# shamim-hussain/egt

Hardware: AMD Instinct MI355X
Metric: graphs/sec EGT fwd+bwd, ZINC-500K padded N=64 (higher is better)
Workload: dtype f32; 1 GPU; zinc500k_n64: attention-block stack (h,e,mask)->(h',e') x Ly, fwd+bwd + param grads; scope=stack, graphs_per_gpu=128, global_batch=128, N=64, Dh=64, De=64, H=8, d=8, Ly=10, parallelism=dp1, grad_allreduce_bytes=740480, backend=none (single process), flat_grad_adopted=True, flat_grad_bound=True, collective_in_graph=False

## Files before the change

egt_amd/csrc/egt_block.hip:

```cpp
#include "egt_common.h"

#include <stdlib.h>
#include <string.h>
#include <vector>

#include "egt_block.h"
#include "egt_tile.h"

#include "egt_block_dev.h"
#include "egt_dma.h"

#include "egt_block_fwd.h"
#include "egt_block_bwd.h"



struct EgtBlockEnv {
  bool no_narrow_fwd, no_narrow_bwd;
  int bwd_mm;
  int bwd_tl, fwd_rows;
  int nrw_fwd_waves, nrw_bwd_waves, nrw_fwd_half;
};
static bool env_flag_raw(const char* name) {
  const char* v = getenv(name);
// ... 109 lines not shown
    P.fwd_nw = r4 ? 4 : 8;
    P.fl = {B * ((N + 4 * P.fwd_nw - 1) / (4 * P.fwd_nw)), 64 * P.fwd_nw, r4 ? lds_r4 : lds_r8};
  } else {
    P.fwd = FwdKernel::tile;
    P.fl = {B * ((N + P.RGF - 1) / P.RGF), 256, lds_tiles + (P.kvl ? lds_kv : 0)};
  }
  P.epi_ok = P.fwd != FwdKernel::tile || P.kvl;

  if (E.bwd_tl >= 4 && E.bwd_tl <= BWD_TL) P.TL = E.bwd_tl;
  else if (DE != 8) {
    const int g = tg > groups ? tg : groups;
    P.TL = (N + g - 1) / g;
  } else if (B * groups <= cus) {
    P.TL = BWD_TL;
    if (N > 8)
      for (int tl = 8; tl < BWD_TL; ++tl)
        if (B * ((N + tl - 1) / tl) <= cus) { P.TL = tl; break; }
  } else P.TL = (N + groups - 1) / groups;
  P.NLR = (N + P.TL - 1) / P.TL;
  P.nwg_bwd = B * P.NLR;
  P.EP = GG::EP;
  if (DE == 8 && !ml && !E.no_narrow_bwd) {
    P.bwd = BwdKernel::narrow;
    P.bwd_nw = E.nrw_bwd_waves == 8 || (E.nrw_bwd_waves != 4 && P.nwg_bwd <= cus && N >= 64) ? 8 : 4;
    P.bl = {P.nwg_bwd, 64 * P.bwd_nw, egt_narrow_bwd_lds(P.bwd_nw)};
  } else if (DE <= 16 && !ml) {
    constexpr int PWR = V4R_RR * (2 * GG::TILE_FLOATS + 256 + 192);
    P.bwd = BwdKernel::v4r;
    P.bl = {P.nwg_bwd, 256,
            ((size_t)(4 * PWR > BWD_PRO_WS ? 4 * PWR : BWD_PRO_WS) + (size_t)BWD_TL * QD_LD + 3 * GG::TILES * 256 + 3 * 2048 + 4) * 4};
  } else if (DE >= 32 && !ml && d->dtype != EGT_BF16) {
    P.bwd = BwdKernel::v5;
    P.mm = E.bwd_mm;
    P.bl = {P.nwg_bwd, 256, ((size_t)V5_AREA(DE) + (size_t)BWD_TL * QD_LD + 3 * ((GG::TILES + 1) / 2) * 512 + 4) * 4};
  } else {
    constexpr int PW = 3 * GG::TILE_FLOATS + 256 + 192;
    P.bwd = BwdKernel::v4;
    P.bl = {P.nwg_bwd, 256,
            ((size_t)(4 * PW > BWD_PRO_WS ? 4 * PW : BWD_PRO_WS) + (size_t)BWD_TL * QD_LD + 3 * ((GG::TILES + 1) / 2) * 512) * 4};
  }

  const size_t rows = (size_t)B * N;
  const int Dh = d->d * d->H;
  size_t o = 0;
  P.v_att = o; o += al(rows * Dh);
  P.stats = o; o += al(rows * BH * 4);
  P.qkvp = o; o += al(rows * QKVP);
  P.pw_sv = o; o += al((size_t)GG::DEP * 16 + 16);
  P.wfrag_sv = o; o += al(Dh <= 64 ? WFRAG_FLOATS : 0);
  P.saved_total = o;
  o = 0;
  P.dvp = o; o += al(rows * 64);
  P.dqp_sz = al(rows * 64 * (size_t)groups);
  P.dkvp_sz = al((size_t)P.nwg_bwd * N * 128);
  P.dqp = o; o += 2 * P.dqp_sz;
  P.dkvp = o; o += 2 * P.dkvp_sz;
  P.common_total = o;
  o = 0;
  P.pw = o; o += al((size_t)GG::DEP * 16 + 16);
  P.epart = o; o += al((size_t)P.nwg_bwd * P.EP);
  {
    const int node_wg = B * ((N + NODE_RC - 1) / NODE_RC);
    const size_t nmax = (size_t)(P.nwg_bwd > node_wg ? P.nwg_bwd : node_wg);
    P.spart = o; o += al(nmax * (5 * Dh));
    P.sbo = o; o += al(nmax * Dh);
  }
  P.wpart = o; o += al((size_t)egt_node_wgrad_chunks((int)rows, 1) * (Dh * 3 * Dh + Dh * Dh));
// ... 158 lines not shown
static int launch_fwd(BlockArgs& a, const BlockPlan& P, hipStream_t st, bool skip_pre) {
  if (!skip_pre) egt_node_launch_pre(a, st);
  if (!(P.epi_ok && node_fused_ok(a))) a.epi = 0;
  a.guard = 0;
  a.RGF = P.RGF;
  switch (P.fwd) {
    case FwdKernel::narrow: egt_narrow_launch_fwd(a, P.fwd_nw, P.fwd_half, P.fl, st); break;
    case FwdKernel::r4:
      if constexpr (DE <= 16) { if (a.bf16) launch_r4<DE, true>(a, P, st); else launch_r4<DE, false>(a, P, st); }
      break;
    case FwdKernel::tile: if (a.bf16) launch_tile_fwd<DE, true>(a, P, st); else launch_tile_fwd<DE, false>(a, P, st); break;
  }
  if (a.epi == 0) egt_node_launch_post(a, st);
  return a.epi;
}

template <int DE>
static void launch_bwd(BlockArgs& a, const BlockPlan& P, hipStream_t st, bool top, BlockArgs* below, BlockArgs* above, bool fuse) {
  static_assert(DE % 16 == 0 || DE == 8, "edge widths of the pair kernels");
  const bool pro = fuse;
  a.pro = 0;
  if (pro) {
    a.pro = top ? 1 : 2;
    a.sbo_n = P.nwg_bwd;
    if (!top) {
      a.up_h = above->h; a.up_nm_g = above->nm_g; a.up_Wqkv = above->Wqkv; a.up_wfrag = above->wfrag; a.up_dh_out = above->dh_out;
      a.up_dqp = above->dqp; a.up_dkvp = above->dkvp; a.up_dqkv_sv = above->dqkv_sv; a.up_spart = above->spart;
      above->spart_n = P.nwg_bwd;
    }
    if (a.prep) egt_node_launch_prep(&a, 1, st);
  } else if (top) {
    egt_node_launch_bwd(a, &a, false, st);
  }
  a.NQP = (a.N + 15) / 16;
  a.guard = 0;
  switch (P.bwd) {
    case BwdKernel::narrow: egt_narrow_launch_bwd(a, P.bwd_nw, P.bl, st); break;
    case BwdKernel::v4r:
      if constexpr (DE <= 16) {
        if (a.bf16) egt_launch_planned<k_block_bwd_v4r<DE, true, V4R_RR>>("k_block_bwd", P.bl, st, a);
        else egt_launch_planned<k_block_bwd_v4r<DE, false, V4R_RR>>("k_block_bwd", P.bl, st, a);
      }
      break;
    case BwdKernel::v5:
      if constexpr (DE >= 32) launch_v5<DE>(a, P, st);
      break;
    case BwdKernel::v4: if (a.bf16) launch_v4<DE, true>(a, P, st); else launch_v4<DE, false>(a, P, st); break;
  }
  if (!pro) egt_node_launch_bwd(a, below, true, st);
  else if (!below) egt_node_launch_bwd(a, nullptr, true, st);
}


extern "C" int egt_block_fwd(const egt_block_desc* desc, const egt_block_params* params,
                             const void* h, const void* e, const uint8_t* key_mask,
                             const void* attn_mask, const uint8_t* rand_mask, void* h_out,
                             void* e_out, void* saved, void* workspace, void* stream) {
  BlockArgs a;
  int rc = fill_block(desc, params, a);
  if (rc) return rc;
  if (!h || !e || !h_out || !e_out || !saved || !workspace)
    EGT_FAIL(EGT_E_NULL, "h/e/h_out/e_out/saved/workspace is NULL");
  if ((desc->flags & EGT_BF_ATTN_MASK) && !attn_mask) EGT_FAIL(EGT_E_NULL, "ATTN_MASK set but attn_mask is NULL");
  const BlockPlan P = plan_block(desc, mask_tensor(desc, rand_mask));
  bind_common(desc, P, a, h, e, key_mask, attn_mask, rand_mask, (float*)saved, (float*)workspace);
  a.h_out = (float*)h_out; a.e_out = (float*)e_out;
  a.epi = 1;
// ... 165 lines not shown
```

egt_amd/csrc/egt_block_bwd.h:

```cpp
#pragma once
#ifndef EGT_NT_BWD_E
#define EGT_NT_BWD_E true
#endif
#ifndef EGT_NT_BWD_DY
#define EGT_NT_BWD_DY false
#endif
#ifndef EGT_NT_BWD_ST
#define EGT_NT_BWD_ST false
#endif

template <int DE, bool ML, bool BF, bool RAG>
__global__ void __launch_bounds__(256, 2) k_block_bwd_v4(BlockArgs a) {
  seed_from_device(a);
  using G = Geo<DE>;
  typedef typename EdgeT<BF>::type ET;
  const ET* e_in = reinterpret_cast<const ET*>(a.e);
  ET* e_o = reinterpret_cast<ET*>(a.e_out);
  const ET* dey_in = reinterpret_cast<const ET*>(a.de_out);
  ET* dex_o = reinterpret_cast<ET*>(a.de);
  (void)e_in; (void)e_o; (void)dey_in; (void)dex_o;
  extern __shared__ __attribute__((aligned(16))) float sm[];
  const int lane = threadIdx.x & 63, wave = threadIdx.x >> 6;
  const int p = lane & 15, q = lane >> 4;
  const int N = a.N, TL = a.TL;
// ... 281 lines not shown
  constexpr int NS = (Geo<DE>::TILES + 1) / 2;
  (void)SPLIT; (void)NS;
  using G = Geo<DE>;
  const float* e_in = a.e;
  const float* dey_in = a.de_out;
  float* dex_o = a.de;
  extern __shared__ __attribute__((aligned(16))) float sm[];
  const int lane = threadIdx.x & 63, wave = __builtin_amdgcn_readfirstlane(threadIdx.x >> 6);
  const int p = lane & 15, q = lane >> 4;
  const int N = a.N, TL = a.TL;
  const int wg = a.xcd ? egt_xcd_remap(blockIdx.x, gridDim.x) : (int)blockIdx.x;
  const int b = wg / a.NLR, lr = wg % a.NLR;
  const int l_begin = lr * TL, l_end = min(N, l_begin + TL), nl = l_end - l_begin;
  const bool gated = (a.flags & EGT_BF_GATE) != 0;
  const bool clip = (a.flags & EGT_BF_CLIP) != 0;
  constexpr int PW = 3 * G::TILE_FLOATS + 256 + 192;
  constexpr int WSLAB = (MM != 0 && NS * 512 > G::TILES * 256) ? NS * 512 : G::TILES * 256;
  constexpr int PW2 = 2 * G::TILE_FLOATS + 256 + 192;
  float* et0 = sm + wave * G::TILE_FLOATS;
  float* et1 = sm + 4 * G::TILE_FLOATS + wave * PW2;
  const int estr = __builtin_amdgcn_readfirstlane((int)(et1 - et0));
  float* dt = et1 + G::TILE_FLOATS;
  float* sc1 = dt + G::TILE_FLOATS;
  float* sc2 = sc1 + 256;
  constexpr int AREA = V5_AREA(DE);
  static_assert(4 * PW == 4 * G::TILE_FLOATS + 4 * PW2 && AREA >= 4 * PW && AREA >= 4 * G::TILE_FLOATS + BWD_PRO_WS, "tile area");
  float* pro_ws = sm + 4 * G::TILE_FLOATS;
  float* qd = sm + AREA;
  float* wsA = qd + TL * QD_LD;
  float* wsB = wsA + WSLAB;
  float* wsD = wsB + WSLAB;
  volatile int* pflag = reinterpret_cast<volatile int*>(wsD + WSLAB);
  if (threadIdx.x < 4) pflag[threadIdx.x] = 0;
  const unsigned et_lds = __builtin_amdgcn_readfirstlane((unsigned)(size_t)et0);
  const unsigned off0 = dma_lane_offset<DE>(lane);
  const int ntile = RAG ? (N + 15) / 16 : N / 16;
  const bool balance = RAG && V5_BALANCE && ntile >= 3 && (ntile & 3) != 0;
  const int T_ = ntile * nl;
  const int t0 = balance ? (wave * T_) >> 2 : 0, t1 = balance ? ((wave + 1) * T_) >> 2 : 0;
  const bool have = balance ? t1 > t0 : wave < ntile;
  const int mt_first = balance ? t0 / nl : wave, mt_last = balance ? (t1 - 1) / nl : ntile - 1, mt_step = balance ? 1 : 4;
  const int r0_first = balance ? t0 - mt_first * nl : 0;
  float Kf[16], Vf[16];
  int kmv = 1;
#define V5_TILE_START(MT_, ROW_)                                                                                    \
  do {                                                                                                              \
    const int m0_ = (MT_) * 16, kv_ = RAG ? min(16, N - m0_) : 16;                                                  \
    if (RAG && kv_ < 16) tile_dma_ragged<DE>(et_lds, e_in + (((size_t)b * N + l_begin + (ROW_)) * N + m0_) * DE, lane, kv_); \
    else tile_dma<DE, EGT_NT_BWD_E>(et_lds, e_in + (((size_t)b * N + l_begin + (ROW_)) * N + m0_) * DE, off0);      \
    const size_t rowm_ = (size_t)b * N + (RAG ? min(m0_ + p, N - 1) : m0_ + p);                                     \
    const float4* kp_ = reinterpret_cast<const float4*>(a.qkvp + rowm_ * QKVP + 64 + q * 16);                       \
    const float4* vp_ = reinterpret_cast<const float4*>(a.qkvp + rowm_ * QKVP + 128 + q * 16);                      \
    _Pragma("unroll") for (int i = 0; i < 4; ++i) {                                                                 \
      const float4 kv4 = kp_[i], vv4 = vp_[i];                                                                      \
      Kf[4*i] = kv4.x; Kf[4*i+1] = kv4.y; Kf[4*i+2] = kv4.z; Kf[4*i+3] = kv4.w;                                     \
      Vf[4*i] = vv4.x; Vf[4*i+1] = vv4.y; Vf[4*i+2] = vv4.z; Vf[4*i+3] = vv4.w;                                     \
    }                                                                                                               \
    kmv = a.km ? (int)a.km[rowm_] : 1;                                                                              \
  } while (0)
  if (have) V5_TILE_START(mt_first, r0_first);
  BwdProRegs proR;
  {
    float4 sv[3];
#pragma unroll
    for (int u = 0; u < 3; ++u) {
      const int i = threadIdx.x + 256 * u, r = i / 40, f = i % 40;
// ... 40 lines not shown
    bwd_node_prologue_finish<DE>(a, pro_ws, qd, b, l_begin, wg, proR);
  }
  PSTAMP(1);
  if constexpr (MM != 0) {
    uint16_t* A16 = reinterpret_cast<uint16_t*>(wsA);
    uint16_t* B16 = reinterpret_cast<uint16_t*>(wsB);
    uint16_t* D16 = reinterpret_cast<uint16_t*>(wsD);
    auto parts = [](float v, uint16_t& hi, uint16_t& lo) {
      const uint32_t h = pk_bf16(v, 0.f) & 0xFFFFu;
      hi = (uint16_t)h;
      lo = (uint16_t)(pk_bf16(v - __uint_as_float(h << 16), 0.f) & 0xFFFFu);
    };
    for (int idx = threadIdx.x; idx < NS * 512; idx += 256) {
      const int i = idx & 7, ln = (idx >> 3) & 63, s_ = idx >> 9, pp = ln & 15, qq = ln >> 4, t = 2 * s_ + (i >> 2);
      const int c = 16 * t + 4 * qq + (i & 3);
      const bool in = t < G::TILES && c < DE;
      const int hd = 2 * (pp >> 2) + (pp & 1);
      uint16_t hi, lo;
      parts(in ? a.pw[c * 16 + pp] : 0.f, hi, lo);
      A16[((s_ * 2 + 0) * 64 + ln) * 8 + i] = hi; A16[((s_ * 2 + 1) * 64 + ln) * 8 + i] = lo;
      parts((in && (pp & 2) == 0) ? a.Wr[hd * DE + c] : 0.f, hi, lo);
      B16[((s_ * 2 + 0) * 64 + ln) * 8 + i] = hi; B16[((s_ * 2 + 1) * 64 + ln) * 8 + i] = lo;
    }
    for (int idx = threadIdx.x; idx < G::TILES * 256; idx += 256) {
      const int u = idx & 3, ln = (idx >> 2) & 63, t = idx >> 8, pp = ln & 15, qq = ln >> 4;
      uint16_t hi, lo;
      parts(a.pw[(16 * t + pp) * 16 + 4 * qq + u], hi, lo);
      D16[(t * 64 + ln) * 8 + u] = hi; D16[(t * 64 + ln) * 8 + 4 + u] = lo;
    }
  }
  float c2r[4];
#pragma unroll
  for (int r = 0; r < 4; ++r) c2r[r] = a.pw[G::DEP * 16 + 4 * q + r];

  v4f accT[G::TILES], accR[G::TILES];
#pragma unroll
  for (int t = 0; t < G::TILES; ++t) { accT[t] = (v4f){0.f, 0.f, 0.f, 0.f}; accR[t] = (v4f){0.f, 0.f, 0.f, 0.f}; }
  float ssum[4] = {0.f, 0.f, 0.f, 0.f};
  __syncthreads();
  PSTAMP(2);

  for (int mt = mt_first; have && mt <= mt_last; mt += mt_step) {
    const int r0 = (balance && mt == mt_first) ? r0_first : 0;
    const int r1 = (balance && mt == mt_last) ? t1 - mt * nl : nl;
    const int m0 = mt * 16, m = m0 + p;
    const int kv = RAG ? min(16, N - m0) : 16;
    const bool kvalid = RAG ? (p < kv) : true;
    if (mt != mt_first) V5_TILE_START(mt, r0);
    float dKa[16], dVa[16];
#pragma unroll
    for (int i = 0; i < 16; ++i) { dKa[i] = 0.f; dVa[i] = 0.f; }
    asm volatile("" : "+v"(kmv));
    const float kadd = kmv == 0 ? -EGT_NEG : 0.0f;
    const int l_first = l_begin + r0, l_stop = l_begin + r1;
    for (int l = l_first; l < l_stop; ++l) {
      const int li = l - l_begin;
      const int lj = l - l_first;
      const size_t rowl = (size_t)b * N + l;
      const size_t pair0 = rowl * N + m0;
      float* et = et0 + (lj & 1) * estr;
      MaskRegs mr{make_float2(1.f, 1.f), 0};
      TileRegs<DE> td;
      tile_gload<DE, EGT_NT_BWD_DY>(td, dey_in + pair0 * DE, lane, kv);
      if (lj == 0) vm_wait<(G::NF4 + 63) / 64>(); else vm_wait<2 * ((G::NF4 + 63) / 64) + 1>();
      SCHED_FENCE();
      float rstd;
      v4f acc = {c2r[0], c2r[1], c2r[2], c2r[3]};
      {
        float4 x[G::TILES];
#pragma unroll
        for (int t = 0; t < G::TILES; ++t) x[t] = frag_read<DE>(et, p, q, t);
        rstd = ln_frags<DE>(x, q, a.ln_eps, (a.flags & EGT_BF_NO_EDGE_LN) == 0);
        if constexpr (MM != 0) {
#pragma unroll
          for (int t = 0; t < G::TILES; ++t) frag_write<DE>(et, p, q, t, x[t]);
          v4f xv[G::TILES];
          Bf8 xh[NS], xl[NS];
#pragma unroll
          for (int t = 0; t < G::TILES; ++t) xv[t] = (v4f){x[t].x, x[t].y, x[t].z, x[t].w};
          split_tiles<G::TILES, SPLIT>(xv, xh, xl);
          acc = bf_gemm<NS, SPLIT>(wsA, 0, lane, xh, xl, acc);
        } else {
#pragma unroll
        for (int t = 0; t < G::TILES; ++t) {
          frag_write<DE>(et, p, q, t, x[t]);
          const float4 w = *reinterpret_cast<const float4*>(wsA + (t * 64 + lane) * 4);
          acc = MFMA(w.x, x[t].x, acc);
          acc = MFMA(w.y, x[t].y, acc);
          acc = MFMA(w.z, x[t].z, acc);
          acc = MFMA(w.w, x[t].w, acc);
        }
        }
      }
      SCHED_FENCE();
      tile_lds_put<DE>(dt, td, lane, kv);
      lds_sync();
      if (l + 1 < l_stop) {
        if (RAG && kv < 16) tile_dma_ragged<DE>(et_lds + (unsigned)(((lj + 1) & 1) * estr * 4), e_in + (pair0 + (size_t)N) * DE, lane, kv);
        else tile_dma<DE, EGT_NT_BWD_E>(et_lds + (unsigned)(((lj + 1) & 1) * estr * 4), e_in + (pair0 + (size_t)N) * DE, off0);
      }
// ... 44 lines not shown
        float xl[2], gl[2], inr[2];
#pragma unroll
        for (int j = 0; j < 2; ++j) {
          const float araw = dots[j] * a.scale;
          float ah = araw;
          inr[j] = 1.0f;
          if (clip) {
            inr[j] = (araw >= a.clip_lo && araw <= a.clip_hi) ? 1.0f : 0.0f;
            ah = fminf(fmaxf(araw, a.clip_lo), a.clip_hi);
          }
          hh[j] = ah + acc[2 * j + 1];
          xl[j] = hh[j];
          gl[j] = acc[2 * j];
        }
        apply_masks<false>(a, kadd, mr, (pair0 + p) * BH, q, xl, gl);
        if (RAG && !kvalid) { xl[0] = xl[1] = -3.0e38f; gl[0] = gl[1] = -3.0e38f; }
#pragma unroll
        for (int j = 0; j < 2; ++j) {
          const float S = __expf(xl[j] - st[4 * j]) * st[4 * j + 1];
          const float g = (gated || (RAG && !kvalid)) ? egt_sigmoid(gl[j]) : 1.0f;
          const float dS = dAd[j] * g;
          const float dGl = gated ? dAd[j] * S * g * (1.0f - g) : 0.f;
          const float dH = S * (dS - st[4 * j + 2]) + dhx[j];
          dA[j] = dH * inr[j] * a.scale;
          at[j] = S * g;
          dge[2 * j] = dGl;
          dge[2 * j + 1] = dH;
        }
      }
#pragma unroll
      for (int r = 0; r < 4; ++r) ssum[r] += dge[r];
      *reinterpret_cast<float4*>(sc1 + p * 16 + 4 * q) = make_float4(dge[0], dge[1], dge[2], dge[3]);
      *reinterpret_cast<float2*>(sc2 + p * 12 + 2 * q) = make_float2(hh[0], hh[1]);
      if (q == 0) sc2[p * 12 + 8] = 1.0f;
      lds_sync();
      SCHED_FENCE();
      if (!(a.guard & 4))
      {
        const float* qr = qd + li * QD_LD;
        const float4* qp = reinterpret_cast<const float4*>(qr + q * 16);
        const float4* dp = reinterpret_cast<const float4*>(qr + 64 + q * 16);
        float dq[16];
#pragma unroll
        for (int i = 0; i < 4; ++i) {
          const float4 u = qp[i], v = dp[i];
          dKa[4*i]   = fmaf(dA[0], u.x, dKa[4*i]);   dKa[4*i+1] = fmaf(dA[1], u.y, dKa[4*i+1]);
          dKa[4*i+2] = fmaf(dA[0], u.z, dKa[4*i+2]); dKa[4*i+3] = fmaf(dA[1], u.w, dKa[4*i+3]);
          dVa[4*i]   = fmaf(at[0], v.x, dVa[4*i]);   dVa[4*i+1] = fmaf(at[1], v.y, dVa[4*i+1]);
          dVa[4*i+2] = fmaf(at[0], v.z, dVa[4*i+2]); dVa[4*i+3] = fmaf(at[1], v.w, dVa[4*i+3]);
        }
#pragma unroll
        for (int k = 0; k < 8; ++k) { dq[2 * k] = dA[0] * Kf[2 * k]; dq[2 * k + 1] = dA[1] * Kf[2 * k + 1]; }
        a.dqp[(((size_t)b * ntile + mt) * N + l) * 64 + lane] = reduce16_keep_own(dq, p);
      }
      SCHED_FENCE();
      if (!(a.guard & 1))
      {
        float bT[4], bR[4];
#pragma unroll
        for (int s = 0; s < 4; ++s) {
          bT[s] = sc1[(q + 4 * s) * 16 + p];
          bR[s] = (p < 9) ? sc2[(q + 4 * s) * 12 + p] : 0.f;
        }
        {
          const int lb = 64 * q + 4 * ((p >> 2) ^ q) + (p & 3);
          const float* eb = et + lb;
          const float* db = dt + lb;
#pragma unroll
          for (int t = 0; t < G::TILES; ++t)
#pragma unroll
            for (int s = 0; s < 4; ++s) {
              accT[t] = MFMA(elem_read_st<DE>(eb, et, p, q, s, t), bT[s], accT[t]);
              accR[t] = MFMA(elem_read_st<DE>(db, dt, p, q, s, t), bR[s], accR[t]);
            }
        }
      }
      lds_sync();
      SCHED_FENCE();
      if (!(a.guard & 2)) {
        float4 dxh[G::TILES];
        float m1 = 0.f, m2 = 0.f;
        Bf8 gB1, gB2;
        if constexpr (MM != 0) {
          const uint32_t h0 = pk_bf16(dge[0], dge[1]), h1 = pk_bf16(dge[2], dge[3]);
          gB1.u[0] = h0; gB1.u[1] = h1; gB1.u[2] = h0; gB1.u[3] = h1;
          gB2.u[0] = pk_bf16(dge[0] - __uint_as_float(h0 << 16), dge[1] - __uint_as_float(h0 & 0xFFFF0000u));
          gB2.u[1] = pk_bf16(dge[2] - __uint_as_float(h1 << 16), dge[3] - __uint_as_float(h1 & 0xFFFF0000u));
          gB2.u[2] = 0u; gB2.u[3] = 0u;
        }
#pragma unroll
        for (int t = 0; t < G::TILES; ++t) {
          const float4 xh = frag_read<DE>(et, p, q, t);
          v4f d = {0.f, 0.f, 0.f, 0.f};
          if constexpr (MM != 0) {
            Bf8 wa, wb;
            wa.q = *reinterpret_cast<const uint4*>(wsD + (t * 64 + lane) * 4);
            d = MFMA_BF(wa.v, gB1.v, d);
            if (SPLIT) {
              wb.u[0] = wa.u[0]; wb.u[1] = wa.u[1]; wb.u[2] = 0u; wb.u[3] = 0u;
              d = MFMA_BF(wb.v, gB2.v, d);
            }
          } else {
          const float4 w = *reinterpret_cast<const float4*>(wsD + (t * 64 + lane) * 4);
          d = MFMA(w.x, dge[0], d);
          d = MFMA(w.y, dge[1], d);
          d = MFMA(w.z, dge[2], d);
          d = MFMA(w.w, dge[3], d);
          }
          dxh[t] = make_float4(d[0], d[1], d[2], d[3]);
          m1 += (d[0] + d[1]) + (d[2] + d[3]);
          m2 = fmaf(d[0], xh.x, m2); m2 = fmaf(d[1], xh.y, m2);
          m2 = fmaf(d[2], xh.z, m2); m2 = fmaf(d[3], xh.w, m2);
        }
        m1 = sum_over_q(m1) * (1.0f / DE);
        m2 = sum_over_q(m2) * (1.0f / DE);
        if (a.flags & EGT_BF_NO_EDGE_LN) { m1 = 0.f; m2 = 0.f; }
        float* orow = dex_o + (pair0 + p) * DE + 4 * q;
#pragma unroll
        for (int t = 0; t < G::TILES; ++t) {
          if (16 * t + 4 * q < DE) {
            const float4 dyv = frag_read<DE>(dt, p, q, t);
            const float4 xh = frag_read<DE>(et, p, q, t);
            float4 o;
            o.x = dyv.x + rstd * (dxh[t].x - m1 - xh.x * m2);
            o.y = dyv.y + rstd * (dxh[t].y - m1 - xh.y * m2);
            o.z = dyv.z + rstd * (dxh[t].z - m1 - xh.z * m2);
            o.w = dyv.w + rstd * (dxh[t].w - m1 - xh.w * m2);
            if (kvalid) { if (EGT_NT_BWD_ST) egt_st4_nt(orow + 16 * t, o); else *reinterpret_cast<float4*>(orow + 16 * t) = o; }
          }
        }
        lds_sync();
      }
      SCHED_FENCE();
    }
    float4* ko = reinterpret_cast<float4*>(a.dkvp + (((((size_t)b * a.NLR + lr) * N + m) * 2 + 0) * 4 + q) * 16);
    float4* vo = reinterpret_cast<float4*>(a.dkvp + (((((size_t)b * a.NLR + lr) * N + m) * 2 + 1) * 4 + q) * 16);
    if (balance && r1 < nl && r0 == 0) {
      while (pflag[wave + 1] == 0) __builtin_amdgcn_s_sleep(1);
      __builtin_amdgcn_fence(__ATOMIC_ACQUIRE, "workgroup");
      if (kvalid) {
#pragma unroll
        for (int i = 0; i < 4; ++i) {
          const float4 kk = ko[i], vv = vo[i];
          dKa[4*i] += kk.x; dKa[4*i+1] += kk.y; dKa[4*i+2] += kk.z; dKa[4*i+3] += kk.w;
          dVa[4*i] += vv.x; dVa[4*i+1] += vv.y; dVa[4*i+2] += vv.z; dVa[4*i+3] += vv.w;
        }
      }
    }
    if (kvalid) {
#pragma unroll
      for (int i = 0; i < 4; ++i) {
        ko[i] = make_float4(dKa[4*i], dKa[4*i+1], dKa[4*i+2], dKa[4*i+3]);
        vo[i] = make_float4(dVa[4*i], dVa[4*i+1], dVa[4*i+2], dVa[4*i+3]);
      }
    }
    if (balance && r0 > 0) {
      __builtin_amdgcn_fence(__ATOMIC_RELEASE, "workgroup");
      asm volatile("s_waitcnt vmcnt(0)" ::: "memory");
      if (lane == 0) pflag[wave] = 1;
    }
  }
#pragma unroll
  for (int r = 0; r < 4; ++r) ssum[r] = row_sum16(ssum[r]);
  __syncthreads();
  float* ep = sm + wave * G::EP;
#pragma unroll
  for (int t = 0; t < G::TILES; ++t)
#pragma unroll
    for (int r = 0; r < 4; ++r) {
      ep[(16 * t + 4 * q + r) * 16 + p] = accT[t][r];
      ep[G::DEP * 16 + 16 + (16 * t + 4 * q + r) * 16 + p] = accR[t][r];
    }
  if (p == 0) {
#pragma unroll
    for (int r = 0; r < 4; ++r) ep[G::DEP * 16 + 4 * q + r] = ssum[r];
  }
  __syncthreads();
  float* out = a.epart + (size_t)wg * G::EP;
  for (int i = threadIdx.x; i < G::EP; i += 256)
    out[i] = (sm[i] + sm[G::EP + i]) + (sm[2 * G::EP + i] + sm[3 * G::EP + i]);
}

template <int DE, bool BF, int R>
__global__ void __launch_bounds__(256, 2) k_block_bwd_v4r(BlockArgs a) {
  seed_from_device(a);
  using G = Geo<DE>;
  typedef typename EdgeT<BF>::type ET;
  const ET* e_in = reinterpret_cast<const ET*>(a.e);
  const ET* dey_in = reinterpret_cast<const ET*>(a.de_out);
  ET* dex_o = reinterpret_cast<ET*>(a.de);
  extern __shared__ __attribute__((aligned(16))) float sm[];
  const int lane = threadIdx.x & 63, wave = threadIdx.x >> 6;
  const int p = lane & 15, q = lane >> 4;
  const int N = a.N, TL = a.TL;
  const int wg = a.xcd ? egt_xcd_remap(blockIdx.x, gridDim.x) : (int)blockIdx.x;
  int b, lr;
  egt_group_order(wg, a.B, a.NLR, N, b, lr, TL);
  const int l_begin = lr * TL, l_end = min(N, l_begin + TL), nl = l_end - l_begin;
  const bool gated = (a.flags & EGT_BF_GATE) != 0;
  const bool clip = (a.flags & EGT_BF_CLIP) != 0;
  constexpr int TF = G::TILE_FLOATS;
  constexpr int PWR = R * (2 * TF + 256 + 192);
  constexpr int WSLAB = G::TILES * 256;
  float* et0 = sm + wave * PWR;
  float* dt0 = et0 + R * TF;
  float* sc10 = dt0 + R * TF;
  float* sc20 = sc10 + R * 256;
  constexpr int AREA = 4 * PWR > BWD_PRO_WS ? 4 * PWR : BWD_PRO_WS;
  static_assert(4 * G::EP <= AREA, "edge partial staging must fit the LDS tile area");
  float* qd = sm + AREA;
  float* wsA = qd + TL * QD_LD;
  float* wsB = wsA + WSLAB;
  float* wsD = wsB + WSLAB;
// ... 303 lines not shown
```

egt_amd/csrc/egt_dma.h:

```cpp
#pragma once
#include "egt_tile.h"

template <int DE>
__device__ __forceinline__ unsigned dma_lane_offset(int lane) {
  if (DE == 64) return (unsigned)((lane >> 4) * 256 + (((lane & 15) ^ swz<64>(lane >> 4)) << 4));
  return (unsigned)(lane * 16);
}
#define EGT_TILE_DMA_BODY(MOD) \
  constexpr int NI = Geo<DE>::NF4 / 64; \
  static_assert(Geo<DE>::NF4 % 64 == 0 && NI >= 1 && NI <= 4, "whole 1 KiB chunks"); \
  unsigned keep, t; \
  constexpr unsigned X = DE == 64 ? 1088u : 1024u; \
  constexpr unsigned X1 = X, X2 = 2 * X, X3 = 3 * X; \
  if (NI == 4) \
    asm volatile( \
        "s_mov_b32 %0, m0\n\ts_mov_b32 m0, %4\n\ts_nop 0\n\tglobal_load_lds_dwordx4 %3, %2" MOD "\n\t" \
        "v_xor_b32 %1, %5, %3\n\ts_add_u32 m0, m0, 1024\n\ts_nop 0\n\tglobal_load_lds_dwordx4 %1, %2" MOD "\n\t" \
        "v_xor_b32 %1, %6, %3\n\ts_add_u32 m0, m0, 1024\n\ts_nop 0\n\tglobal_load_lds_dwordx4 %1, %2" MOD "\n\t" \
        "v_xor_b32 %1, %7, %3\n\ts_add_u32 m0, m0, 1024\n\ts_nop 0\n\tglobal_load_lds_dwordx4 %1, %2" MOD "\n\t" \
        "s_mov_b32 m0, %0" \
        : "=&s"(keep), "=&v"(t) : "s"(src), "v"(off0), "s"(lds), "i"(X1), "i"(X2), "i"(X3) : "memory", "scc"); \
  else if (NI == 3) \
    asm volatile( \
        "s_mov_b32 %0, m0\n\ts_mov_b32 m0, %4\n\ts_nop 0\n\tglobal_load_lds_dwordx4 %3, %2" MOD "\n\t" \
        "v_xor_b32 %1, %5, %3\n\ts_add_u32 m0, m0, 1024\n\ts_nop 0\n\tglobal_load_lds_dwordx4 %1, %2" MOD "\n\t" \
        "v_xor_b32 %1, %6, %3\n\ts_add_u32 m0, m0, 1024\n\ts_nop 0\n\tglobal_load_lds_dwordx4 %1, %2" MOD "\n\t" \
        "s_mov_b32 m0, %0" \
        : "=&s"(keep), "=&v"(t) : "s"(src), "v"(off0), "s"(lds), "i"(X1), "i"(X2) : "memory", "scc"); \
  else if (NI == 2) \
    asm volatile( \
        "s_mov_b32 %0, m0\n\ts_mov_b32 m0, %4\n\ts_nop 0\n\tglobal_load_lds_dwordx4 %3, %2" MOD "\n\t" \
        "v_xor_b32 %1, %5, %3\n\ts_add_u32 m0, m0, 1024\n\ts_nop 0\n\tglobal_load_lds_dwordx4 %1, %2" MOD "\n\t" \
        "s_mov_b32 m0, %0" \
        : "=&s"(keep), "=&v"(t) : "s"(src), "v"(off0), "s"(lds), "i"(X1) : "memory", "scc"); \
  else \
    asm volatile( \
        "s_mov_b32 %0, m0\n\ts_mov_b32 m0, %3\n\ts_nop 0\n\tglobal_load_lds_dwordx4 %2, %1" MOD "\n\t" \
        "s_mov_b32 m0, %0" \
        : "=&s"(keep) : "s"(src), "v"(off0), "s"(lds) : "memory"); \
  (void)t;
template <int DE, bool NT = false>
__device__ __forceinline__ void tile_dma(unsigned lds, const float* src, unsigned off0) {
  if (NT) { EGT_TILE_DMA_BODY(" nt") } else { EGT_TILE_DMA_BODY("") }
}
#undef EGT_TILE_DMA_BODY
template <int DE>
__device__ __forceinline__ void tile_dma_ragged(unsigned lds, const float* src, int lane, int rows_valid) {
  using G = Geo<DE>;
  constexpr int NI = G::NF4 / 64;
#pragma unroll
  for (int i = 0; i < NI; ++i) {
    const int f = 64 * i + lane, row = f / G::NSLOT, slot = f % G::NSLOT;
    const int rc = min(row, rows_valid - 1);
    const unsigned off = (unsigned)((rc * G::NSLOT + (DE == 64 ? (slot ^ swz<64>(row)) : slot)) << 4);
    unsigned keep;
    asm volatile("s_mov_b32 %0, m0\n\ts_mov_b32 m0, %3\n\ts_nop 0\n\tglobal_load_lds_dwordx4 %2, %1\n\ts_mov_b32 m0, %0"
                 : "=&s"(keep) : "s"(src), "v"(off), "s"(lds + 1024u * i) : "memory");
  }
}
template <int N_>
__device__ __forceinline__ void vm_wait() { asm volatile("s_waitcnt vmcnt(%0)" :: "i"(N_) : "memory"); }

template <int DE>
__device__ __forceinline__ float elem_read_st(const float* lane_base, const float* tl, int p, int q, int s, int t) {
  if (DE == 64) return lane_base[256 * s + 16 * (t ^ s)];
  return elem_read<DE>(tl, q + 4 * s, 16 * t + p);
}

__device__ __forceinline__ void tile_prefetch(unsigned lds_dump, const float* src, unsigned lane_off) {
  unsigned keep;
  asm volatile("s_mov_b32 %0, m0\n\ts_mov_b32 m0, %3\n\ts_nop 0\n\tglobal_load_lds_dword %2, %1\n\ts_mov_b32 m0, %0"
               : "=&s"(keep) : "s"(src), "v"(lane_off), "s"(lds_dump) : "memory");
}
```

egt_amd/csrc/egt_node.hip:

```cpp
#include <stdlib.h>

#include "egt_block.h"

#define LDP 4

__device__ __forceinline__ float sum16(float v) { return row_sum16(v); }

__device__ __forceinline__ v4f mm_xw(const float* xs, int ld, const float* W, int ldw,
                                     int K, int p, int q, bool colok, v4f acc) {
#pragma unroll 4
  for (int t = 0; t < K; t += 4) {
    const float bv = colok ? W[(size_t)(t + q) * ldw + p] : 0.f;
    acc = MFMA(xs[p * ld + t + q], bv, acc);
  }
  return acc;
}
__device__ __forceinline__ v4f mm_xwt(const float* xs, int ld, const float* W, int ldw,
                                      int K, int p, int q, bool colok, v4f acc) {
#pragma unroll 4
  for (int t = 0; t < K; t += 4) {
    const float bv = colok ? W[(size_t)p * ldw + t + q] : 0.f;
    acc = MFMA(xs[p * ld + t + q], bv, acc);
  }
  return acc;
// ... 347 lines not shown
  Stg<2> sWo;
  Stg<1> sV, sX;
  float4 gq[3];
  float dho[4], gmm[4];
  if (DV) {
    stg_issue_weight(sWo, x.wo_a, Dh * Dh / 4);
    stg_issue_rows(sV, x.dv_v_att + row0 * Dh, Dh, nr, nrp);
  }
  if (PRE) {
    stg_issue_weight(sWq, x.wq_a, Dh * D3 / 4);
    stg_issue_rows(sX, a.h + row0 * Dh, Dh, nr, nrp);
    {
      const int row = 4 * wave + q;
#pragma unroll
      for (int i = 0; i < 4; ++i) {
        const int c = p + 16 * i;
        const bool ok = row < nr && c < Dh;
        dho[i] = a.dh_out[ok ? (row0 + row) * Dh + c : row0 * Dh];
        gmm[i] = a.nm_g[c < Dh ? c : 0];
      }
    }
    const int U = nrp * 48;
#pragma unroll
    for (int u = 0; u < 3; ++u) {
      const int i = t + u * 512, r = i / 48, pos4 = (i % 48) * 4, sx = pos4 >> 6;
      const bool ok = i < U && r < nr;
      const int rc = ok ? r : 0;
      float4 acc4 = make_float4(0.f, 0.f, 0.f, 0.f);
      const int np = sx == 0 ? a.NQP : a.NLR;
      const float* base = sx == 0 ? a.dqp + ((size_t)b * a.NQP * N + r0 + rc) * 64 + pos4
                                  : a.dkvp + (((size_t)b * a.NLR * N + r0 + rc) * 2 + (sx - 1)) * 64 + (pos4 & 63);
      const size_t pstride = sx == 0 ? (size_t)N * 64 : (size_t)N * 128;
      if (NP > 0) {
#pragma unroll
        for (int pi = 0; pi < NP; ++pi) {
          const float4 w = *reinterpret_cast<const float4*>(base + pi * pstride);
          acc4.x += w.x; acc4.y += w.y; acc4.z += w.z; acc4.w += w.w;
        }
      } else {
        const int npmax = max(a.NQP, a.NLR);
#pragma unroll 4
        for (int pi = 0; pi < npmax; ++pi) {
          const float4 w = *reinterpret_cast<const float4*>(base + min(pi, np - 1) * pstride);
          const float f = pi < np ? 1.0f : 0.0f;
          acc4.x = fmaf(w.x, f, acc4.x); acc4.y = fmaf(w.y, f, acc4.y);
          acc4.z = fmaf(w.z, f, acc4.z); acc4.w = fmaf(w.w, f, acc4.w);
        }
      }
      gq[u] = sel4(ok, acc4);
    }
  } else {
    stg_issue_rows(sX, x.dv_dh_src + row0 * Dh, Dh, nr, nrp);
  }
  if (DV) { stg_pin(sWo); stg_pin(sV); }
  stg_pin(sX);
  if (PRE) {
    stg_pin(sWq);
#pragma unroll
    for (int u = 0; u < 3; ++u) pin4(gq[u]);
  }
  if (DV) {
    stg_commit_weight(sWo, wo, ld, x.dv_Wo, x.wo_al != 0, Dh, Dh);
    stg_commit_rows(sV, vs, ld, Dh, nr, nrp);
  }
  if (PRE) {
    stg_commit_weight(sWq, ws, ld3, a.Wqkv, x.wq_al != 0, Dh, D3);
    stg_commit_rows(sX, xs, ld, Dh, nr, nrp);
    const int U = nrp * 48;
#pragma unroll
    for (int u = 0; u < 3; ++u) {
// ... 411 lines not shown
  if (n > 40) return false;
  const BlockArgs& a = as[0];
  size_t lds = lds_rows(a.Dh, 1) + (size_t)a.Dh * (3 * a.Dh + LDP) * 4;
  if (lds < 1024) lds = 1024;
  if (n <= 16) launch_pre_stack<16>(as, n, lds, st);
  else launch_pre_stack<40>(as, n, lds, st);
  return true;
}

void egt_node_launch_post(BlockArgs& a, hipStream_t st) {
  const size_t lds = lds_rows(a.Dh, 1) + (size_t)a.Dh * (a.Dh + LDP) * 4;
  EGT_LAUNCH("k_node_post", k_node_post, dim3(a.B * node_chunks(a)), dim3(512), lds, st, a);
}

void egt_node_launch_bwd(BlockArgs& a, const BlockArgs* dv_layer, bool do_pre, hipStream_t st) {
  NodeBwdArgs x{};
  auto down16 = [](const float* p) { return reinterpret_cast<const float*>(reinterpret_cast<uintptr_t>(p) & ~(uintptr_t)15); };
  x.wq_a = down16(a.Wqkv); x.wq_al = x.wq_a == a.Wqkv;
  if (dv_layer) {
    x.wo_a = down16(dv_layer->Wo); x.wo_al = x.wo_a == dv_layer->Wo;
    x.dv_Wo = dv_layer->Wo; x.dv_v_att = dv_layer->v_att; x.dv_dh_src = a.dh_out;
    x.dv_stats = dv_layer->stats; x.dv_dvp = dv_layer->dvp; x.dv_sbo = dv_layer->sbo;
  }
  const int Dh = a.Dh, ld = Dh + LDP, ld3 = 3 * Dh + LDP;
  size_t lds = ((size_t)4 * NODE_RC * ld + NODE_RC + 4 * NODE_RC * 8 + (size_t)Dh * ld) * 4;
  if (do_pre) lds += ((size_t)NODE_RC * ld3 + (size_t)Dh * ld3) * 4;
  const bool prep = !do_pre && a.prep;
  const dim3 grid(a.B * node_chunks(a) + (prep ? 1 : 0));
#define NODE_BWD(PRE_, DV_, NP_, NAME)                                                                     \
  do {                                                                                                 \
    EGT_MAX_LDS_ONCE(k_node_bwd<PRE_, DV_, NP_>); \
    EGT_LAUNCH(NAME, (k_node_bwd<PRE_, DV_, NP_>), grid, dim3(512), lds, st, a, x);                    \
  } while (0)
  const bool np4 = a.NQP == 4 && a.NLR == 4;
  if (!do_pre) NODE_BWD(false, true, 0, "k_node_bwd_top");
  else if (dv_layer) { if (np4) NODE_BWD(true, true, 4, "k_node_bwd"); else NODE_BWD(true, true, 0, "k_node_bwd"); }
  else { if (np4) NODE_BWD(true, false, 4, "k_node_bwd"); else NODE_BWD(true, false, 0, "k_node_bwd"); }
#undef NODE_BWD
}

static int wgrad_rows_per_wg(int rows, int layers) {
  int per_layer = (2 * egt_device_cus()) / (layers > 0 ? layers : 1);
  if (per_layer < 1) per_layer = 1;
  const int r = (((rows + per_layer - 1) / per_layer + 31) / 32) * 32;
  return r < WG_ROWS ? WG_ROWS : r;
}
int egt_node_wgrad_chunks(int rows, int layers) { const int r = wgrad_rows_per_wg(rows, layers); return (rows + r - 1) / r; }

void egt_node_launch_wgrads(BlockArgs* as, int n, hipStream_t st) {
  WGradArgs wa{};
  const BlockArgs& a0 = as[0];
  wa.rows = a0.B * a0.N; wa.Dh = a0.Dh; wa.ln_eps = a0.ln_eps; wa.rows_per_wg = wgrad_rows_per_wg(wa.rows, n);
  for (int l = 0; l < n; ++l) {
    const BlockArgs& a = as[l];
    wa.L[l] = WGradLayer{a.h, a.nm_g, a.nm_b, a.dqkv_sv, a.v_att, a.dh_out, a.wpart};
  }
  const int Dh = a0.Dh;
  const size_t lds = ((size_t)3 * 32 * (Dh + 16) + (size_t)32 * (3 * Dh + 16)) * 4;
  const dim3 grid(egt_node_wgrad_chunks(wa.rows, n), n);
  for (int l = 0; l < n; ++l) as[l].wpart_n = (int)grid.x;
  if (Dh == 64) EGT_LAUNCH("k_node_wgrads", k_node_wgrads<true>, grid, dim3(512), lds, st, wa);
  else EGT_LAUNCH("k_node_wgrads", k_node_wgrads<false>, grid, dim3(512), lds, st, wa);
}

void egt_node_launch_prep(BlockArgs* as, int n, hipStream_t st) {
  for (int l0 = 0; l0 < n; l0 += PREP_MAX_LAYERS) {
    const int nl = n - l0 < PREP_MAX_LAYERS ? n - l0 : PREP_MAX_LAYERS;
// ... 48 lines not shown
```

Baseline: 79470 graphs/s.

## Reduce dQ partials inside the v5 backward kernel and specialize DE=64 accR path

The v5 edge backward kernel now accumulates each row's dQ contributions in registers across all key tiles. It sums them across the four waves through LDS staging and writes one dQ partial per row, instead of one per key tile. The node backward kernel is told NQP=1, so it reads a single dQ partial rather than summing four. For DE=64 with the MM path, the accR MFMA accumulation is replaced by 4x4x1 MFMAs plus a scalar row-sum, and the c2 constants are staged in LDS. The change also relaxes a vm_wait count and adds a few register-pinning asm hints; the cost is extra registers for dQacc and more LDS use.

```diff
diff --git a/egt_amd/csrc/egt_block.hip b/egt_amd/csrc/egt_block.hip
--- a/egt_amd/csrc/egt_block.hip
+++ b/egt_amd/csrc/egt_block.hip
@@ -165,7 +165,7 @@
   } else if (DE >= 32 && !ml && d->dtype != EGT_BF16) {
     P.bwd = BwdKernel::v5;
     P.mm = E.bwd_mm;
-    P.bl = {P.nwg_bwd, 256, ((size_t)V5_AREA(DE) + (size_t)BWD_TL * QD_LD + 3 * ((GG::TILES + 1) / 2) * 512 + 4) * 4};
+    P.bl = {P.nwg_bwd, 256, ((size_t)V5_AREA(DE) + (size_t)BWD_TL * QD_LD + 3 * ((GG::TILES + 1) / 2) * 512 + 4 + 16) * 4};
   } else {
     constexpr int PW = 3 * GG::TILE_FLOATS + 256 + 192;
     P.bwd = BwdKernel::v4;
@@ -390,7 +390,7 @@
   } else if (top) {
     egt_node_launch_bwd(a, &a, false, st);
   }
-  a.NQP = (a.N + 15) / 16;
+  a.NQP = P.bwd == BwdKernel::v5 ? 1 : (a.N + 15) / 16;
   a.guard = 0;
   switch (P.bwd) {
     case BwdKernel::narrow: egt_narrow_launch_bwd(a, P.bwd_nw, P.bl, st); break;
diff --git a/egt_amd/csrc/egt_block_bwd.h b/egt_amd/csrc/egt_block_bwd.h
--- a/egt_amd/csrc/egt_block_bwd.h
+++ b/egt_amd/csrc/egt_block_bwd.h
@@ -337,6 +337,8 @@
   float* wsD = wsB + WSLAB;
   volatile int* pflag = reinterpret_cast<volatile int*>(wsD + WSLAB);
   if (threadIdx.x < 4) pflag[threadIdx.x] = 0;
+  constexpr bool C2L = RAG || MM != 0;
+  float* c2s = wsD + WSLAB + 4;
   const unsigned et_lds = __builtin_amdgcn_readfirstlane((unsigned)(size_t)et0);
   const unsigned off0 = dma_lane_offset<DE>(lane);
   const int ntile = RAG ? (N + 15) / 16 : N / 16;
@@ -443,11 +445,21 @@
   float c2r[4];
 #pragma unroll
   for (int r = 0; r < 4; ++r) c2r[r] = a.pw[G::DEP * 16 + 4 * q + r];
+  if (C2L && p == 0 && wave == 0) *reinterpret_cast<float4*>(c2s + 4 * q) = make_float4(c2r[0], c2r[1], c2r[2], c2r[3]);
 
-  v4f accT[G::TILES], accR[G::TILES];
-#pragma unroll
-  for (int t = 0; t < G::TILES; ++t) { accT[t] = (v4f){0.f, 0.f, 0.f, 0.f}; accR[t] = (v4f){0.f, 0.f, 0.f, 0.f}; }
+  constexpr bool R4 = DE == 64 && MM != 0;
+  constexpr int NR = R4 ? 2 : G::TILES;
+  v4f accT[G::TILES], accR[NR];
+  float brs = 0.f;
+  (void)brs;
+#pragma unroll
+  for (int t = 0; t < G::TILES; ++t) accT[t] = (v4f){0.f, 0.f, 0.f, 0.f};
+#pragma unroll
+  for (int t = 0; t < NR; ++t) accR[t] = (v4f){0.f, 0.f, 0.f, 0.f};
   float ssum[4] = {0.f, 0.f, 0.f, 0.f};
+  float dQacc[BWD_TL];
+#pragma unroll
+  for (int i = 0; i < BWD_TL; ++i) dQacc[i] = 0.f;
   __syncthreads();
   PSTAMP(2);
 
@@ -473,10 +485,11 @@
       MaskRegs mr{make_float2(1.f, 1.f), 0};
       TileRegs<DE> td;
       tile_gload<DE, EGT_NT_BWD_DY>(td, dey_in + pair0 * DE, lane, kv);
-      if (lj == 0) vm_wait<(G::NF4 + 63) / 64>(); else vm_wait<2 * ((G::NF4 + 63) / 64) + 1>();
+      if (lj == 0) vm_wait<(G::NF4 + 63) / 64>(); else vm_wait<2 * ((G::NF4 + 63) / 64)>();
       SCHED_FENCE();
       float rstd;
       v4f acc = {c2r[0], c2r[1], c2r[2], c2r[3]};
+      if constexpr (C2L) { const float4 c4 = *reinterpret_cast<const float4*>(c2s + 4 * q); acc = (v4f){c4.x, c4.y, c4.z, c4.w}; }
       {
         float4 x[G::TILES];
 #pragma unroll
@@ -587,7 +600,7 @@
       for (int r = 0; r < 4; ++r) ssum[r] += dge[r];
       *reinterpret_cast<float4*>(sc1 + p * 16 + 4 * q) = make_float4(dge[0], dge[1], dge[2], dge[3]);
       *reinterpret_cast<float2*>(sc2 + p * 12 + 2 * q) = make_float2(hh[0], hh[1]);
-      if (q == 0) sc2[p * 12 + 8] = 1.0f;
+      if (!R4 && q == 0) sc2[p * 12 + 8] = 1.0f;
       lds_sync();
       SCHED_FENCE();
       if (!(a.guard & 4))
@@ -606,7 +619,7 @@
         }
 #pragma unroll
         for (int k = 0; k < 8; ++k) { dq[2 * k] = dA[0] * Kf[2 * k]; dq[2 * k + 1] = dA[1] * Kf[2 * k + 1]; }
-        a.dqp[(((size_t)b * ntile + mt) * N + l) * 64 + lane] = reduce16_keep_own(dq, p);
+        dQacc[li] += reduce16_keep_own(dq, p);
       }
       SCHED_FENCE();
       if (!(a.guard & 1))
@@ -615,7 +628,7 @@
 #pragma unroll
         for (int s = 0; s < 4; ++s) {
           bT[s] = sc1[(q + 4 * s) * 16 + p];
-          bR[s] = (p < 9) ? sc2[(q + 4 * s) * 12 + p] : 0.f;
+          bR[s] = (!R4 && p < 9) ? sc2[(q + 4 * s) * 12 + p] : 0.f;
         }
         {
           const int lb = 64 * q + 4 * ((p >> 2) ^ q) + (p & 3);
@@ -626,8 +639,20 @@
 #pragma unroll
             for (int s = 0; s < 4; ++s) {
               accT[t] = MFMA(elem_read_st<DE>(eb, et, p, q, s, t), bT[s], accT[t]);
-              accR[t] = MFMA(elem_read_st<DE>(db, dt, p, q, s, t), bR[s], accR[t]);
+              if constexpr (!R4) accR[t] = MFMA(elem_read_st<DE>(db, dt, p, q, s, t), bR[s], accR[t]);
             }
+        }
+        if constexpr (R4) {
+          int la = lane;
+          asm volatile("" : "+v"(la));
+          const float* hb = sc2 + (la & 3);
+#pragma unroll
+          for (int k = 0; k < 16; ++k) {
+            const float av = dt[64 * k + (la ^ (4 * k))];
+            accR[0] = __builtin_amdgcn_mfma_f32_4x4x1f32(av, hb[12 * k], accR[0], 0, 0, 0);
+            accR[1] = __builtin_amdgcn_mfma_f32_4x4x1f32(av, hb[12 * k + 4], accR[1], 0, 0, 0);
+            brs += av;
+          }
         }
       }
       lds_sync();
@@ -688,8 +713,10 @@
       }
       SCHED_FENCE();
     }
-    float4* ko = reinterpret_cast<float4*>(a.dkvp + (((((size_t)b * a.NLR + lr) * N + m) * 2 + 0) * 4 + q) * 16);
-    float4* vo = reinterpret_cast<float4*>(a.dkvp + (((((size_t)b * a.NLR + lr) * N + m) * 2 + 1) * 4 + q) * 16);
+    int ms = m;
+    asm volatile("" : "+v"(ms));
+    float4* ko = reinterpret_cast<float4*>(a.dkvp + (((((size_t)b * a.NLR + lr) * N + ms) * 2 + 0) * 4 + q) * 16);
+    float4* vo = reinterpret_cast<float4*>(a.dkvp + (((((size_t)b * a.NLR + lr) * N + ms) * 2 + 1) * 4 + q) * 16);
     if (balance && r1 < nl && r0 == 0) {
       while (pflag[wave + 1] == 0) __builtin_amdgcn_s_sleep(1);
       __builtin_amdgcn_fence(__ATOMIC_ACQUIRE, "workgroup");
@@ -724,16 +751,35 @@
 #pragma unroll
     for (int r = 0; r < 4; ++r) {
       ep[(16 * t + 4 * q + r) * 16 + p] = accT[t][r];
-      ep[G::DEP * 16 + 16 + (16 * t + 4 * q + r) * 16 + p] = accR[t][r];
-    }
+      if constexpr (!R4) ep[G::DEP * 16 + 16 + (16 * t + 4 * q + r) * 16 + p] = accR[t][r];
+    }
+  if constexpr (R4) {
+    float* rp = ep + G::DEP * 16 + 16;
+#pragma unroll
+    for (int h2 = 0; h2 < 2; ++h2)
+#pragma unroll
+      for (int i = 0; i < 4; ++i) rp[(4 * (lane >> 2) + i) * 16 + 4 * h2 + (lane & 3)] = accR[h2][i];
+    rp[lane * 16 + 8] = brs;
+#pragma unroll
+    for (int c = 9; c < 16; ++c) rp[lane * 16 + c] = 0.f;
+  }
   if (p == 0) {
 #pragma unroll
     for (int r = 0; r < 4; ++r) ep[G::DEP * 16 + 4 * q + r] = ssum[r];
   }
+  static_assert(4 * G::EP + 4 * BWD_TL * 64 <= AREA, "edge partial + dQ staging must fit the LDS tile area");
+  float* dqs = sm + 4 * G::EP;
+#pragma unroll
+  for (int i = 0; i < BWD_TL; ++i) dqs[(wave * BWD_TL + i) * 64 + lane] = dQacc[i];
   __syncthreads();
   float* out = a.epart + (size_t)wg * G::EP;
-  for (int i = threadIdx.x; i < G::EP; i += 256)
+  int tid = threadIdx.x;
+  asm volatile("" : "+v"(tid));
+  for (int i = tid; i < G::EP; i += 256)
     out[i] = (sm[i] + sm[G::EP + i]) + (sm[2 * G::EP + i] + sm[3 * G::EP + i]);
+  float* dqo = a.dqp + ((size_t)b * N + l_begin) * 64;
+  for (int i = tid; i < nl * 64; i += 256)
+    dqo[i] = ((dqs[i] + dqs[BWD_TL * 64 + i]) + dqs[2 * BWD_TL * 64 + i]) + dqs[3 * BWD_TL * 64 + i];
 }
 
 template <int DE, bool BF, int R>
diff --git a/egt_amd/csrc/egt_dma.h b/egt_amd/csrc/egt_dma.h
--- a/egt_amd/csrc/egt_dma.h
+++ b/egt_amd/csrc/egt_dma.h
@@ -48,6 +48,7 @@
 __device__ __forceinline__ void tile_dma_ragged(unsigned lds, const float* src, int lane, int rows_valid) {
   using G = Geo<DE>;
   constexpr int NI = G::NF4 / 64;
+  asm volatile("" : "+v"(lane));
 #pragma unroll
   for (int i = 0; i < NI; ++i) {
     const int f = 64 * i + lane, row = f / G::NSLOT, slot = f % G::NSLOT;
diff --git a/egt_amd/csrc/egt_node.hip b/egt_amd/csrc/egt_node.hip
--- a/egt_amd/csrc/egt_node.hip
+++ b/egt_amd/csrc/egt_node.hip
@@ -403,10 +403,12 @@
                                   : a.dkvp + (((size_t)b * a.NLR * N + r0 + rc) * 2 + (sx - 1)) * 64 + (pos4 & 63);
       const size_t pstride = sx == 0 ? (size_t)N * 64 : (size_t)N * 128;
       if (NP > 0) {
+        const bool one = sx == 0 && a.NQP == 1;
 #pragma unroll
         for (int pi = 0; pi < NP; ++pi) {
-          const float4 w = *reinterpret_cast<const float4*>(base + pi * pstride);
-          acc4.x += w.x; acc4.y += w.y; acc4.z += w.z; acc4.w += w.w;
+          const float4 w = *reinterpret_cast<const float4*>(base + (one ? 0 : pi) * pstride);
+          const bool in = pi == 0 || !one;
+          acc4.x += in ? w.x : 0.f; acc4.y += in ? w.y : 0.f; acc4.z += in ? w.z : 0.f; acc4.w += in ? w.w : 0.f;
         }
       } else {
         const int npmax = max(a.NQP, a.NLR);
@@ -884,7 +886,7 @@
     EGT_MAX_LDS_ONCE(k_node_bwd<PRE_, DV_, NP_>); \
     EGT_LAUNCH(NAME, (k_node_bwd<PRE_, DV_, NP_>), grid, dim3(512), lds, st, a, x);                    \
   } while (0)
-  const bool np4 = a.NQP == 4 && a.NLR == 4;
+  const bool np4 = (a.NQP == 4 || a.NQP == 1) && a.NLR == 4;
   if (!do_pre) NODE_BWD(false, true, 0, "k_node_bwd_top");
   else if (dv_layer) { if (np4) NODE_BWD(true, true, 4, "k_node_bwd"); else NODE_BWD(true, true, 0, "k_node_bwd"); }
   else { if (np4) NODE_BWD(true, false, 4, "k_node_bwd"); else NODE_BWD(true, false, 0, "k_node_bwd"); }
```

Result: no change. 79680 graphs/s (median of 4 runs) (+0.3%).
